# TimingSpace/MVOScaleRecovery

Hardware: AMD Instinct MI355X
Metric: frames/sec scale-recovery, KITTI-00 flow (~2k feats/frame), 1/2/4/8 GPU (higher is better)
Workload: dtype f64

## Files before the change

### mvoscalerecovery_amd/csrc/mvosr_kernels.hip

```cpp
#include <hip/hip_runtime.h>
#include <math.h>
#include <stdint.h>
#include <stdlib.h>
#include <string.h>

#include "../../include/mvosr.h"
#include "mvosr_device.hpp"
#include "mvosr_host.hpp"

namespace mvosr {

#ifdef MVOSR_STAMPS
#define MVOSR_STAMP(i) do { if (threadIdx.x == 0 && stamps) stamps[i] = __builtin_amdgcn_s_memtime(); } while (0)
#define MVOSR_STAMP_DECL unsigned long long stamps[12] = {0,0,0,0,0,0,0,0,0,0,0,0};
#define MVOSR_STAMP_ARG , unsigned long long *stamps = nullptr
#define MVOSR_STAMP_PASS , stamps
#define MVOSR_RSTAMP(i) do { if (stamps) stamps[i] = __builtin_amdgcn_s_memtime(); } while (0)
#else
#define MVOSR_RSTAMP(i) do {} while (0)
#define MVOSR_STAMP(i) do {} while (0)
#define MVOSR_STAMP_DECL
#define MVOSR_STAMP_ARG
#define MVOSR_STAMP_PASS
#endif

struct LdsPlan {
    uint32_t p, y, c, hist, red, misc, total;
// ... 22 lines not shown
    uint32_t *sel;
    int *hist;
    double *red;
    int *misc;
};
__device__ __forceinline__ Smem carve(char *base, int n, int waves) {
    const LdsPlan p = lds_plan(n, waves);
    Smem s;
    s.P = reinterpret_cast<double2 *>(base + p.p);
    s.Y = reinterpret_cast<double *>(base + p.y);
    s.c16 = reinterpret_cast<uint16_t *>(base + p.c);
    s.c32 = reinterpret_cast<uint32_t *>(base + p.c);
    s.sel = reinterpret_cast<uint32_t *>(base + p.c);
    s.hist = reinterpret_cast<int *>(base + p.hist);
    s.red = reinterpret_cast<double *>(base + p.red);
    s.misc = reinterpret_cast<int *>(base + p.misc);
    return s;
}

enum { M_WCNT = 0 , M_LIST = 16, M_MEDLO = 18, M_MEDHI = 20  };


constexpr int kTC = 2;


typedef double dvec2 __attribute__((ext_vector_type(2)));
__device__ __forceinline__ double2 stream_load2(const double2 *p) {
    const dvec2 v = __builtin_nontemporal_load(reinterpret_cast<const dvec2 *>(p));
    double2 r; r.x = v.x; r.y = v.y;
    return r;
}
__device__ __forceinline__ double stream_load(const double *p) {
    return __builtin_nontemporal_load(p);
}

template <int B>
struct TriChunk {
    TriIds q[kTC];
    template <bool STREAM = false>
    __device__ __forceinline__ void load(const int32_t *tri, int64_t begin, int count, int base, int tid) {
#pragma unroll
        for (int k = 0; k < kTC; ++k) {
            const int t = base + k * B + tid;
            if (t < count) {
                if constexpr (STREAM) {
                    const int32_t *p = tri + 3 * begin + 3 * t;
                    q[k].a = __builtin_nontemporal_load(p); q[k].b = __builtin_nontemporal_load(p + 1); q[k].c = __builtin_nontemporal_load(p + 2);
                } else {
                    q[k] = load_tri(tri + 3 * begin, t);
                }
            }
        }
    }
};

struct VoteFlags { bool f0, f1, f2; };
__device__ __forceinline__ VoteFlags vote_flags(bool pa, bool pb, bool pc, bool fixed) {
    const bool pb1 = pb & !fixed, pb2 = pb & fixed;
    VoteFlags r;
    r.f0 = pa | pb; r.f1 = pa | pb1 | pc; r.f2 = pb2 | pc;
    return r;
}
__device__ __forceinline__ int tri_rows(const int64_t *off, const int32_t *cnt, int64_t f) {
    return cnt ? cnt[f] : (int)(off[f + 1] - off[f]);
}

template <int WAVES, int SC>
__device__ __forceinline__ int phase_vote(const Smem &s, int n, const double *gx, const double *gy, const double *gz,
                                          const double *gv, const int32_t *tri1, int64_t t1_begin, int t1_count,
                                          double cp, double sp, int32_t *g_counters, int &bad,
                                          const int32_t *tri2, int64_t t2_begin, int t2_count, TriChunk<WAVES * kWave> &next,
                                          bool fixed MVOSR_STAMP_ARG) {
    constexpr int B = WAVES * kWave;
    const int tid = threadIdx.x;
    const int npad2 = (n + 1) >> 1;
    TriChunk<B> tc;
    tc.template load<true>(tri1, t1_begin, t1_count, 0, tid);
    const double2 *gy2 = reinterpret_cast<const double2 *>(gy);
    const double2 *gz2 = reinterpret_cast<const double2 *>(gz);
    const double2 *gv2 = reinterpret_cast<const double2 *>(gv);
    double2 *sY2 = reinterpret_cast<double2 *>(s.Y);
    const uint32_t ones = ((uint32_t)(kCounterBias + 1) << 16) | (uint32_t)(kCounterBias + 1);
    for (int i0 = tid; i0 < npad2; i0 += 2 * B) {
        const int i1 = i0 + B;
        const bool two = i1 < npad2;
        const double2 ya = stream_load2(gy2 + i0), za = stream_load2(gz2 + i0), va = stream_load2(gv2 + i0);
        double2 yb = ya, zb = za, vb = va;
        if (two) { yb = stream_load2(gy2 + i1); zb = stream_load2(gz2 + i1); vb = stream_load2(gv2 + i1); }
        double2 yr, p0, p1;
        yr.x = ya.x * cp - za.x * sp;  yr.y = ya.y * cp - za.y * sp;
        p0.x = va.x; p0.y = ya.x * sp + za.x * cp;
        p1.x = va.y; p1.y = ya.y * sp + za.y * cp;
        sY2[i0] = yr; s.P[2 * i0] = p0; s.P[2 * i0 + 1] = p1; s.c32[i0] = ones;
        if (two) {
            yr.x = yb.x * cp - zb.x * sp;  yr.y = yb.y * cp - zb.y * sp;
            p0.x = vb.x; p0.y = yb.x * sp + zb.x * cp;
            p1.x = vb.y; p1.y = yb.y * sp + zb.y * cp;
            sY2[i1] = yr; s.P[2 * i1] = p0; s.P[2 * i1 + 1] = p1; s.c32[i1] = ones;
        }
    }
    __syncthreads();
    MVOSR_STAMP(1);

    const int w = wave_id(), lane = lane_id();
    const int begin = w * (SC * kWave);
    double xs[SC];
#pragma unroll
    for (int k = 0; k < SC; ++k) {
        const int i = begin + k * kWave + lane;
        xs[k] = (gx && i < n) ? stream_load(gx + i) : 0.0;
    }

    TriChunk<B> tn;
    for (int base = 0; base < t1_count; base += kTC * B) {
        const bool more = base + kTC * B < t1_count;
        if (more) tn.template load<true>(tri1, t1_begin, t1_count, base + kTC * B, tid);
        double2 vp[kTC][3];
        bool vok[kTC];
#pragma unroll
        for (int k = 0; k < kTC; ++k) {
            const TriIds q = tc.q[k];
            vok[k] = base + k * B + tid < t1_count;
            if (vok[k] && ((unsigned)q.a >= (unsigned)n || (unsigned)q.b >= (unsigned)n || (unsigned)q.c >= (unsigned)n)) { bad = 1; vok[k] = false; }
            if (vok[k]) { vp[k][0] = s.P[q.a]; vp[k][1] = s.P[q.b]; vp[k][2] = s.P[q.c]; }
        }
#pragma unroll
        for (int k = 0; k < kTC; ++k) {
            if (!vok[k]) continue;
            const TriIds q = tc.q[k];
            const double2 p0 = vp[k][0], p1 = vp[k][1], p2 = vp[k][2];
            const bool pa = (p0.x - p1.x) * (p0.y - p1.y) > 0.0;
            const bool pb = (p0.x - p2.x) * (p0.y - p2.y) > 0.0;
            const bool pc = (p1.x - p2.x) * (p1.y - p2.y) > 0.0;
            const VoteFlags vf = vote_flags(pa, pb, pc, fixed);
            const bool f0 = vf.f0, f1 = vf.f1, f2 = vf.f2;
            atomicAdd(&s.c32[q.a >> 1], (f0 ? 0xFFFFFFFFu : 1u) << ((q.a & 1) * 16));
            atomicAdd(&s.c32[q.b >> 1], (f1 ? 0xFFFFFFFFu : 1u) << ((q.b & 1) * 16));
            atomicAdd(&s.c32[q.c >> 1], (f2 ? 0xFFFFFFFFu : 1u) << ((q.c & 1) * 16));
        }
        if (more) tc = tn;
    }
    if (tri2) next.load(tri2, t2_begin, t2_count, 0, tid);
    __syncthreads();
    MVOSR_STAMP(2);

    unsigned keepmask = 0u;
    double yk[SC], zk[SC];
    int cnt = 0;
#pragma unroll
    for (int k = 0; k < SC; ++k) {
        const int i = begin + k * kWave + lane;
        bool keep = false;
        yk[k] = 0.0; zk[k] = 0.0;
        if (i < n) {
            const int c = (int)s.c16[i] - kCounterBias;
            keep = c >= 0;
            if (g_counters) g_counters[i] = c;
            yk[k] = s.Y[i];
            zk[k] = s.P[i].y;
        }
        if (keep) keepmask |= 1u << k;
        cnt += __popcll(__ballot(keep));
    }
    if (lane == 0) s.misc[M_WCNT + w] = cnt;
    __syncthreads();
// ... 110 lines not shown
    for (int lo = kNpBufSize; lo < n; lo += kNpBufSize) res += np_pairwise_chunk_stream(st, min(kNpBufSize, n - lo));
    return res;
}

template <bool INLINE>
__device__ int pitch_reference_impl(double x0, double y0, double z0, double x1, double y1, double z1,
                                    double x2, double y2, double z2, double thr_deg,
                                    double &nx, double &ny, double &nz, double &pitch) {
    int r = 0;
    if (!plane_normal(x0, y0, z0, x1, y1, z1, x2, y2, z2, nx, ny, nz)) r |= 4;
    const double len2 = (nx * nx + ny * ny) + nz * nz;
    const double len = sqrt(len2);
    const double uy = ny / len;
    pitch = asin(-uy) * 180.0 / 3.141592653589793;
    if (pitch < thr_deg) r |= 1;
    if (pitch >= thr_deg) r |= 2;
    return r;
}
__device__ __attribute__((noinline)) int pitch_reference_cold(double x0, double y0, double z0, double x1, double y1, double z1,
                                                              double x2, double y2, double z2, double thr_deg) {
    double nx, ny, nz, pitch;
    return pitch_reference_impl<false>(x0, y0, z0, x1, y1, z1, x2, y2, z2, thr_deg, nx, ny, nz, pitch);
}
template <bool FULL>
__device__ __forceinline__ int pitch_reference(double x0, double y0, double z0, double x1, double y1, double z1,
                                               double x2, double y2, double z2, double thr_deg,
                                               double &nx, double &ny, double &nz, double &pitch) {
    if constexpr (FULL) return pitch_reference_impl<true>(x0, y0, z0, x1, y1, z1, x2, y2, z2, thr_deg, nx, ny, nz, pitch);
    else { nx = ny = nz = pitch = 0.0; return pitch_reference_cold(x0, y0, z0, x1, y1, z1, x2, y2, z2, thr_deg); }
}

struct SelectResult {
    double height_level;
    int n_pitch, n_tri_valid;
    int singular, bad;
    int n_steep;
    int near;
};

enum { MODE_HOT = 0, MODE_EXACT = 1, MODE_FULL = 2 };

struct PitchTest {
    double thr_deg;
    double s2_hi, s2_lo;
};

template <bool FULL>
__device__ __forceinline__ int classify_triangle(double x0, double y0, double z0, double x1, double y1, double z1,
                                                 double x2, double y2, double z2, double h, const PitchTest &pt,
                                                 double *g_normals, double *g_pitch, double *g_heights, int64_t tg) {
    bool is_flat = false, is_steep = false, is_singular = false;
    bool decided = false;
    if constexpr (!FULL) {
        const double e1x = x1 - x0, e1y = y1 - y0, e1z = z1 - z0;
        const double e2x = x2 - x0, e2y = y2 - y0, e2z = z2 - z0;
        const double cx = __builtin_fma(e1y, e2z, -(e1z * e2y));
        const double cy = __builtin_fma(e1z, e2x, -(e1x * e2z));
        const double cz = __builtin_fma(e1x, e2y, -(e1y * e2x));
        const double tx = x0 * cx, ty = y0 * cy, tz = z0 * cz;
        const double det = (tx + ty) + tz;
        const double mag = (fabs(tx) + fabs(ty)) + fabs(tz);
        const double c2 = __builtin_fma(cz, cz, __builtin_fma(cy, cy, cx * cx));
        const double q2 = cy * cy;
        const double sy = cy * det;
        const bool safe = fabs(det) > 1e-9 * mag;
        is_flat = safe & (sy > 0.0) & (q2 > pt.s2_hi * c2);
        is_steep = safe & ((sy <= 0.0) | (q2 < pt.s2_lo * c2));
        decided = is_flat | is_steep;
    }
    if (!decided) {
        double nx, ny, nz, pitch;
        const int r = pitch_reference<FULL>(x0, y0, z0, x1, y1, z1, x2, y2, z2, pt.thr_deg, nx, ny, nz, pitch);
        is_singular = r & 4;
        is_flat = r & 1;
        is_steep = r & 2;
        if constexpr (FULL) {
            if (g_normals) { double *o = g_normals + 3 * tg; o[0] = nx; o[1] = ny; o[2] = nz; }
            if (g_pitch) g_pitch[tg] = pitch;
            if (g_heights) g_heights[tg] = h;
        }
    }
    return (is_flat ? 1 : 0) | (is_steep ? 2 : 0) | (is_singular ? 4 : 0) | (decided ? 0 : 8);
}

template <bool FULL, class Fetch>
struct SteepStream {
    const int32_t *tri;
    const int32_t *order;
    int t2n;
    const PitchTest &pt;
    Fetch fetch;
    int t_next;
    unsigned long long mask;
    double h;
    __device__ __forceinline__ void refill() {
// ... 99 lines not shown
            *slot = c0 == 0 ? val[0] : *slot + val[0];
        }
        __syncthreads();
    }
    res = *slot;
    __syncthreads();
    return (0.0 + res) / (double)n_steep;
}

struct LdsFetch {
    const double2 *P; const double *Y; int n_valid;
    __device__ __forceinline__ bool operator()(const TriIds q, double &x0, double &y0, double &z0, double &x1, double &y1, double &z1,
                                               double &x2, double &y2, double &z2) const {
        if ((unsigned)q.a >= (unsigned)n_valid || (unsigned)q.b >= (unsigned)n_valid || (unsigned)q.c >= (unsigned)n_valid) return false;
        const double2 p0 = P[q.a], p1 = P[q.b], p2 = P[q.c];
        x0 = p0.x; z0 = p0.y; x1 = p1.x; z1 = p1.y; x2 = p2.x; z2 = p2.y;
        y0 = Y[q.a]; y1 = Y[q.b]; y2 = Y[q.c];
        return true;
    }
};

constexpr double kLevelGuard = 1e-12;

template <int WAVES, int MODE, int FW = 1>
__device__ __forceinline__ SelectResult phase_select(const Smem &s, int n_valid, const int32_t *tri2, int64_t t2_begin,
                                                     int t2_count, TriChunk<WAVES * kWave> &tc, PitchTest pt,
                                                     double *g_normals, double *g_pitch, double *g_heights, int bad_in,
                                                     double *scratch, int scratch_cap MVOSR_STAMP_ARG) {
    constexpr int B = WAVES * kWave;
    constexpr bool FULL = MODE == MODE_FULL;
    const int tid = threadIdx.x;
    unsigned long long flat = 0ull;
    unsigned long long flat_hi = 0ull;
    double hsum = 0.0, hcnt = 0.0, habs = 0.0;
    int npitch = 0, singular = 0, bad = 0;
    int undecided = 0;
    if (t2_count > 64 * FW * B) { bad = 1; t2_count = 0; }
    auto test_triangle = [&](int t, int kk, const TriIds q) {
    if ((unsigned)q.a >= (unsigned)n_valid || (unsigned)q.b >= (unsigned)n_valid || (unsigned)q.c >= (unsigned)n_valid) { bad = 1; return; }
    const double2 p0 = s.P[q.a], p1 = s.P[q.b], p2 = s.P[q.c];
    const double y0 = s.Y[q.a], y1 = s.Y[q.b], y2 = s.Y[q.c];
    const double x0 = p0.x, z0 = p0.y, x1 = p1.x, z1 = p1.y, x2 = p2.x, z2 = p2.y;
    const double h = MODE == MODE_HOT ? (y0 + y1) + y2 : div3((y0 + y1) + y2);
    const int r = classify_triangle<FULL>(x0, y0, z0, x1, y1, z1, x2, y2, z2, h, pt, g_normals, g_pitch, g_heights, t2_begin + t);
    const bool is_flat = r & 1, is_steep = r & 2;
    if (r & 4) singular = 1;
    if constexpr (MODE == MODE_HOT) { if (r & 8) undecided = 1; }
    if (is_steep) { hsum += h; hcnt += 1.0; if constexpr (MODE == MODE_HOT) habs += fabs(h); }
    if (is_flat) {
        if (FW == 1 || kk < 64) flat |= 1ull << (kk & 63); else flat_hi |= 1ull << (kk & 63);
        ++npitch;
    }
    };
    TriChunk<B> tn;
    for (int base = 0; base < t2_count; base += kTC * B) {
        const bool more = base + kTC * B < t2_count;
        if (more) tn.load(tri2, t2_begin, t2_count, base + kTC * B, tid);
#pragma unroll
        for (int k = 0; k < kTC; ++k) {
            const int t = base + k * B + tid;
            if (t < t2_count) test_triangle(t, base / B + k, tc.q[k]);
        }
        if (more) tc = tn;
    }
    const bool in_regs = t2_count <= kTC * B;
    if (!in_regs && t2_count > 0) tc.template load<true>(tri2, t2_begin, t2_count, 0, tid);
    if constexpr (MODE == MODE_HOT) block_sum3<WAVES>(hsum, hcnt, habs, s.red + R_SEL_H * 2 * WAVES, s.red + R_SEL_ABS * 2 * WAVES);
    else block_sum2<WAVES>(hsum, hcnt, s.red + R_SEL_H * 2 * WAVES);
    MVOSR_STAMP(4);
    SelectResult r;
    double hl = hsum / hcnt;
    const double guard = kLevelGuard * (habs / hcnt);
    if constexpr (MODE != MODE_HOT) {
        if (scratch && (int)hcnt + kNpMaxLeaves <= scratch_cap)
            hl = exact_height_level_block<WAVES, FULL>(tri2 + 3 * t2_begin, t2_count, (int)hcnt, pt, LdsFetch{s.P, s.Y, n_valid}, nullptr,
                                                       scratch, s.misc + M_WCNT, s.red + R_MISC * 2 * WAVES);
        else
            hl = exact_height_level<FULL>(tri2 + 3 * t2_begin, t2_count, (int)hcnt, pt, LdsFetch{s.P, s.Y, n_valid});
    }
    int ntv = 0, near = undecided;
    auto mark_triangle = [&](int kk, int qa, int qb, int qc) {
        const unsigned long long fw = (FW == 1 || kk < 64) ? flat : flat_hi;
        if (!((fw >> (kk & 63)) & 1ull)) return;
        const double y0 = s.Y[qa], y1 = s.Y[qb], y2 = s.Y[qc];
        const double h = MODE == MODE_HOT ? (y0 + y1) + y2 : div3((y0 + y1) + y2);
        if constexpr (MODE == MODE_HOT) { if (fabs(h - hl) <= guard) near = 1; }
        if (h > hl) {
            ++ntv;
            atomicOr(&s.sel[qa >> 5], 1u << (qa & 31));
            atomicOr(&s.sel[qb >> 5], 1u << (qb & 31));
            atomicOr(&s.sel[qc >> 5], 1u << (qc & 31));
        }
    };
    for (int base = 0; base < t2_count; base += kTC * B) {
        const bool more = base + kTC * B < t2_count;
        if (more) tn.template load<true>(tri2, t2_begin, t2_count, base + kTC * B, tid);
#pragma unroll
        for (int k = 0; k < kTC; ++k) {
            if (base + k * B + tid < t2_count) mark_triangle(base / B + k, tc.q[k].a, tc.q[k].b, tc.q[k].c);
        }
        if (more) tc = tn;
    }
    bad |= bad_in;
    int sn = singular | (near << 16);
    block_sum4i<WAVES>(npitch, ntv, sn, bad, s.red + R_SEL_CNT * 2 * WAVES);
    singular = sn & 0xFFFF;
    r.near = sn >> 16;
    MVOSR_STAMP(5);
    r.height_level = MODE == MODE_HOT ? hl / 3.0 : hl;
    r.n_steep = (int)hcnt;
    r.n_pitch = npitch; r.n_tri_valid = ntv; r.singular = singular; r.bad = bad;
    return r;
}

struct RoadResult {
    double height;
    int status;
    int n_sel, n_kept, n_modes, mode_left, mode_right;
    double mean, std, skew, median;
};

__device__ __forceinline__ bool dropped_by_single(double y, int bin, const Bits192 &single, int first_single) {
    bool d = false;
#pragma unroll
// ... 477 lines not shown
        if (a.o.stats) { double *st = a.o.stats + 4 * f; st[0] = st[1] = st[2] = st[3] = nan(""); }
    }
}

template <int MODE, bool LIST, class Body>
__device__ __forceinline__ void for_frames(const KArgs &a, Body body) {
    if constexpr (MODE == MODE_EXACT) {
        if (a.redo_pass) {
            const int count = a.redo[0];
            for (int i = blockIdx.x; i < count; i += gridDim.x) {
                body((int64_t)a.redo[1 + i]);
                __syncthreads();
            }
            return;
        }
    }
    if constexpr (LIST) {
        if ((int)blockIdx.x < *a.cls_cnt) body((int64_t)a.cls_list[blockIdx.x]);
        return;
    }
    body(a.first_frame + blockIdx.x);
}

template <int WAVES, int SC, int MODE, bool LIST = false>
__global__ __launch_bounds__(WAVES *kWave, (WAVES == 8 && MODE == MODE_HOT ? 6 : 1)) void scale_frames_kernel(const KArgs a) {
    extern __shared__ __attribute__((aligned(16))) char smem[];
    for_frames<MODE, LIST>(a, [&](const int64_t f) {
    constexpr int B = WAVES * kWave;
    MVOSR_STAMP_DECL
    MVOSR_STAMP(11);
    const int n = a.b.feat_cnt[f];
    const int64_t off = a.b.feat_off[f];
    const int64_t t1b = a.b.tri1_off[f], t2b = a.b.tri2_off[f];
    const int t1n = tri_rows(a.b.tri1_off, a.b.tri1_cnt, f), t2n = tri_rows(a.b.tri2_off, a.b.tri2_cnt, f);
    const Smem s = carve(smem, n, WAVES);
#ifdef MVOSR_STAMPS
    if (n < 0) return;
#endif
    MVOSR_STAMP(0);
#ifdef MVOSR_STAMPS
    if (threadIdx.x == 0) {
        stamps[10] = (unsigned long long)__builtin_amdgcn_s_getreg((31 << 11) | 4) | ((unsigned long long)__builtin_amdgcn_s_getreg((31 << 11) | 20) << 32);
    }
#endif

    RoadResult R;
    R.height = nan(""); R.n_sel = R.n_kept = R.n_modes = 0; R.mode_left = R.mode_right = -1;
    R.mean = R.std = R.skew = R.median = nan("");
    if (early_frame_exit(a, f, n, t2n)) return;
    int bad = 0;
    TriChunk<B> tc2;
    const int nvalid = phase_vote<WAVES, SC>(s, n, a.b.x + off, a.b.y + off, a.b.z + off, a.b.v + off, a.b.tri1, t1b, t1n,
                                             a.P.cos_pitch, a.P.sin_pitch,
                                             a.o.vote_counters ? a.o.vote_counters + off : nullptr, bad,
                                             a.b.tri2, t2b, t2n, tc2, a.P.vote_mode == MVOSR_VOTE_FIXED MVOSR_STAMP_PASS);
    const bool mask_mismatch = a.b.n2_expected && a.b.n2_expected[f] != nvalid;

    SelectResult S;
    S.height_level = nan(""); S.n_pitch = S.n_tri_valid = 0; S.singular = 0; S.bad = 1; S.n_steep = 0; S.near = 0;
    const bool too_many_rows = t1n > kMaxVoteRows;
    if (!mask_mismatch && !too_many_rows)
        S = phase_select<WAVES, MODE>(s, nvalid, a.b.tri2, t2b, t2n, tc2, a.pt, a.o.tri_normals, a.o.tri_pitch_deg,
                                      a.o.tri_heights, bad, a.ysel ? a.ysel + off : nullptr, n MVOSR_STAMP_PASS);
    frame_tail<WAVES, MODE>(a, s, f, off, nvalid, mask_mismatch || too_many_rows, S, R);
    MVOSR_STAMP(9);
#ifdef MVOSR_STAMPS
    if (threadIdx.x == 0 && a.o.hist) { unsigned long long *d = reinterpret_cast<unsigned long long *>(a.o.hist + f * 2 * kBins); for (int i = 0; i < 12; ++i) d[i] = stamps[i]; }
#endif
    });
}

struct DenseWs { double2 *P2; double *Y2; };

__host__ __device__ inline uint32_t dense_lds_bytes(int n, int waves) {
    const uint32_t npad = (uint32_t)((n + 1) & ~1);
    return align16(2u * npad + 16u) + align16(4u * ((uint32_t)(n + 31) / 32u)) + 8u * (uint32_t)(kRedSlots * 2 * waves) + 4u * 32u;
}

template <int DW, bool FUSED>
__device__ __forceinline__ int phase_vote_dense(uint32_t *c32, int *misc, int n, const double *gx, const double *gy, const double *gz,
                                                const double *gv, const int32_t *tri1, int64_t t1_begin, int t1_count,
                                                double cp, double sp, int32_t *g_counters, int &bad,
                                                double2 *P2, double *Y2, bool fixed) {
    constexpr int B = DW * kWave;
    const int tid = threadIdx.x, w = wave_id(), lane = lane_id();
// ... 83 lines not shown
    RoadResult R;
    R.height = nan(""); R.n_sel = R.n_kept = R.n_modes = 0; R.mode_left = R.mode_right = -1;
    R.mean = R.std = R.skew = R.median = nan("");
    if (early_frame_exit(a, f, n, t2n)) return;
    const uint32_t npad = (uint32_t)((n + 1) & ~1);
    Smem s;
    s.c32 = reinterpret_cast<uint32_t *>(smem);
    s.c16 = reinterpret_cast<uint16_t *>(smem);
    s.sel = reinterpret_cast<uint32_t *>(smem + align16(2u * npad + 16u));
    s.red = reinterpret_cast<double *>(smem + align16(2u * npad + 16u) + align16(4u * ((uint32_t)(n + 31) / 32u)));
    s.misc = reinterpret_cast<int *>(s.red + kRedSlots * 2 * DW);
    s.hist = nullptr;
    s.P = da.ws.P2 + off;
    s.Y = da.ws.Y2 + off;
    for (int i = tid; i < (n + 31) / 32; i += B) s.sel[i] = 0u;
    int bad = 0;
    const int nvalid = phase_vote_dense<DW, true>(s.c32, s.misc, n, a.b.x + off, a.b.y + off, a.b.z + off, a.b.v + off, a.b.tri1, t1b, t1n,
                                              a.P.cos_pitch, a.P.sin_pitch, a.o.vote_counters ? a.o.vote_counters + off : nullptr, bad,
                                              da.ws.P2 + off, da.ws.Y2 + off, a.P.vote_mode == MVOSR_VOTE_FIXED);
    const bool mask_mismatch = a.b.n2_expected && a.b.n2_expected[f] != nvalid;
    SelectResult S;
    S.height_level = nan(""); S.n_pitch = S.n_tri_valid = 0; S.singular = 0; S.bad = 1; S.n_steep = 0; S.near = 0;
    if (!mask_mismatch) {
        TriChunk<B> tc2;
        tc2.load(a.b.tri2, t2b, t2n, 0, tid);
        S = phase_select<DW, MODE, 2>(s, nvalid, a.b.tri2, t2b, t2n, tc2, a.pt, a.o.tri_normals, a.o.tri_pitch_deg,
                                      a.o.tri_heights, bad, nullptr, 0);
    }
    frame_tail<DW, MODE>(a, s, f, off, nvalid, mask_mismatch, S, R);
    });
}

template <int DW, int MODE>
__global__ __launch_bounds__(DW *kWave) void scale_frames_dense_feat_kernel(const DenseArgs da) {
    extern __shared__ __attribute__((aligned(16))) char smem[];
    const KArgs &a = da.k;
    for_frames<MODE, false>(a, [&](const int64_t f) {
    constexpr int B = DW * kWave;
    constexpr bool FULL = MODE == MODE_FULL;
    const int tid = threadIdx.x, w = wave_id(), lane = lane_id();
    const int n = a.b.feat_cnt[f];
    const int64_t off = a.b.feat_off[f];
    const int64_t t1b = a.b.tri1_off[f], t2b = a.b.tri2_off[f];
    const int t1n = tri_rows(a.b.tri1_off, a.b.tri1_cnt, f), t2n = tri_rows(a.b.tri2_off, a.b.tri2_cnt, f);
    RoadResult R;
    R.height = nan(""); R.n_sel = R.n_kept = R.n_modes = 0; R.mode_left = R.mode_right = -1;
    R.mean = R.std = R.skew = R.median = nan("");
// ... 574 lines not shown
    const int nvalid = phase_vote_dense<DW, false>(c32, misc, n, nullptr, a.b.y + off, a.b.z + off, a.b.v + off, a.b.tri1, t1b, t1n,
                                               a.P.cos_pitch, a.P.sin_pitch, a.o.vote_counters + off, bad,
                                               nullptr, nullptr, a.P.vote_mode == MVOSR_VOTE_FIXED);
    int b0 = bad, b1 = 0, b2 = 0, b3 = 0;
    block_sum4i<DW>(b0, b1, b2, b3, red + R_MISC * 2 * DW);
    if (threadIdx.x == 0) {
        if (a.o.counts) a.o.counts[f * MVOSR_N_COUNTS + MVOSR_CNT_VALID] = nvalid;
        if (a.o.status) a.o.status[f] = b0 ? MVOSR_ST_ERR_MASK : MVOSR_ST_MODE;
    }
}

template <int WAVES, int SC>
__global__ __launch_bounds__(WAVES *kWave) void outlier_vote_kernel(const KArgs a) {
    extern __shared__ __attribute__((aligned(16))) char smem[];
    const int64_t f = a.first_frame + blockIdx.x;
    const int n = a.b.feat_cnt[f];
    if (n <= 0) { if (threadIdx.x == 0 && a.o.counts) a.o.counts[f * MVOSR_N_COUNTS + MVOSR_CNT_VALID] = 0; return; }
    const int64_t off = a.b.feat_off[f];
    const int64_t t1b = a.b.tri1_off[f];
    const int t1n = tri_rows(a.b.tri1_off, a.b.tri1_cnt, f);
    const Smem s = carve(smem, n, WAVES);
    int bad = 0;
    MVOSR_STAMP_DECL
    TriChunk<WAVES * kWave> unused;
    const int nvalid = phase_vote<WAVES, SC>(s, n, nullptr, a.b.y + off, a.b.z + off, a.b.v + off, a.b.tri1, t1b, t1n,
                                             a.P.cos_pitch, a.P.sin_pitch, a.o.vote_counters + off, bad, nullptr, 0, 0, unused,
                                             a.P.vote_mode == MVOSR_VOTE_FIXED MVOSR_STAMP_PASS);
    int b0 = bad | (t1n > kMaxVoteRows ? 1 : 0), b1 = 0, b2 = 0, b3 = 0;
    block_sum4i<WAVES>(b0, b1, b2, b3, s.red + R_MISC * 2 * WAVES);
    if (threadIdx.x == 0) {
        if (a.o.counts) a.o.counts[f * MVOSR_N_COUNTS + MVOSR_CNT_VALID] = nvalid;
        if (a.o.status) a.o.status[f] = b0 ? MVOSR_ST_ERR_MASK : MVOSR_ST_MODE;
    }
}

constexpr int kMaxWindow = 64;
struct MedianArgs {
    const double *raw; double *out; int64_t n; int window; int n_queue;
    int n_blocks; int64_t base_len, extra, stride;
    double queue[kMaxWindow];
};
__device__ __forceinline__ double median_seq_at(const MedianArgs &a, int64_t i) {
    if (a.n_blocks <= 1) return a.raw[i];
    const int64_t head = a.extra * (a.base_len + 1);
    int64_t r, j;
    if (i < head) { r = i / (a.base_len + 1); j = i - r * (a.base_len + 1); }
    else { const int64_t k = i - head; r = a.extra + k / a.base_len; j = k - (r - a.extra) * a.base_len; }
// ... 28 lines not shown
template <typename K>
static int prepare_kernel(K kernel, size_t lds) {
    hipError_t e = hipFuncSetAttribute(reinterpret_cast<const void *>(kernel), hipFuncAttributeMaxDynamicSharedMemorySize, (int)lds);
    if (e != hipSuccess) return set_hip_error("hipFuncSetAttribute(MaxDynamicSharedMemorySize)", e);
    return MVOSR_OK;
}

static PitchTest make_pitch_test(double thr_deg) {
    PitchTest pt;
    pt.thr_deg = thr_deg;
    if (thr_deg < -1.0 && thr_deg > -89.9) {
        const double sn = sin(-thr_deg * 3.141592653589793 / 180.0);
        pt.s2_hi = sn * sn * (1.0 + 1e-9);
        pt.s2_lo = sn * sn * (1.0 - 1e-9);
    } else {
        pt.s2_hi = INFINITY;
        pt.s2_lo = -INFINITY;
    }
    return pt;
}

constexpr int kClassHeader = 4;
constexpr int kWaves1Max = 320, kWaves4Max = 1152;
constexpr int kClassThr0 = kWaves1Max, kClassThr1 = 1024;
constexpr int64_t kClassMinFrames = 2048;
constexpr int32_t kClassHintMagic = 0x4d56;
constexpr int kClassifyWaves = 16;
struct ClassArgs {
    const int32_t *feat_cnt;
    int64_t first_frame, n_frames;
    int32_t *hdr;
    int32_t *lists;
    int64_t stride;
    int32_t *redo;
    int grid[3];
};

__host__ __device__ inline int size_class_of(int n) { return n <= kClassThr0 ? 0 : (n <= kClassThr1 ? 1 : 2); }

__global__ __launch_bounds__(kClassifyWaves *kWave) void classify_frames_kernel(const ClassArgs c) {
    __shared__ int wcnt[kClassifyWaves][3];
    __shared__ int bbase[3];
    const int64_t i = blockIdx.x * (int64_t)blockDim.x + threadIdx.x;
    const int lane = threadIdx.x & (kWave - 1), w = threadIdx.x / kWave;
    int cls = -1;
    int32_t f = 0;
    if (i < c.n_frames) {
        f = (int32_t)(c.first_frame + i);
        cls = size_class_of(c.feat_cnt[f]);
    }
    const uint64_t m0 = __ballot(cls == 0), m1 = __ballot(cls == 1), m2 = __ballot(cls == 2);
    if (lane == 0) { wcnt[w][0] = __popcll(m0); wcnt[w][1] = __popcll(m1); wcnt[w][2] = __popcll(m2); }
    __syncthreads();
    if (threadIdx.x < 3) {
        int tot = 0;
        for (int ww = 0; ww < kClassifyWaves; ++ww) tot += wcnt[ww][threadIdx.x];
        bbase[threadIdx.x] = tot ? atomicAdd(c.hdr + threadIdx.x, tot) : 0;
    }
    __syncthreads();
    if (cls < 0) return;
    const uint64_t m = cls == 0 ? m0 : (cls == 1 ? m1 : m2);
    int pos = bbase[cls] + __popcll(m & ((1ull << lane) - 1ull));
    for (int ww = 0; ww < w; ++ww) pos += wcnt[ww][cls];
    if (pos < c.grid[cls]) c.lists[cls * c.stride + pos] = f;
    else c.redo[1 + atomicAdd(c.redo, 1)] = f;
}

static int pick_waves(int requested, int max_feat) {
    if (requested == 1 || requested == 4 || requested == 8 || requested == 16) return requested;
    if (max_feat <= kWaves1Max) return 1;
    if (max_feat <= kWaves4Max) return 4;
    if (max_feat <= 2048 || 2 * (int64_t)lds_plan(max_feat, 8).total <= (int64_t)g_max_dyn_lds) return 8;
    return 16;
}
static int variant_capacity(int waves, int sc) { return waves * sc * kWave; }
static int lds_capacity_features() {
    int lo = 1, hi = variant_capacity(16, 8);
    while (lo < hi) {
        const int mid = (lo + hi + 1) / 2;
        if ((int64_t)lds_plan(mid, 16).total <= (int64_t)g_max_dyn_lds) lo = mid; else hi = mid - 1;
    }
    return lo;
}

static int check_common(mvosr_ctx *ctx, const mvosr_params *p, const mvosr_batch *b, const mvosr_outputs *o) {
    if (!ctx || !p || !b || !o) return set_error(MVOSR_ERR_ARG, "null argument");
    if (b->n_frames < 0 || !b->feat_off || !b->feat_cnt) return set_error(MVOSR_ERR_ARG, "batch without frames/offsets");
    if (b->max_feat < 0) return set_error(MVOSR_ERR_ARG, "max_feat < 0");
    return MVOSR_OK;
}

static int check_fit(const mvosr_batch *b, int waves, int sc, size_t lds) {
    if ((int64_t)lds > (int64_t)g_max_dyn_lds)
        return set_error(MVOSR_ERR_TOO_LARGE, "frame of %d features needs %zu B of LDS (> %d)", b->max_feat, lds, g_max_dyn_lds);
    if (b->max_feat > variant_capacity(waves, sc))
        return set_error(MVOSR_ERR_TOO_LARGE, "%d features exceed what %d wavefronts per frame handle (%d)", b->max_feat, waves,
                         variant_capacity(waves, sc));
    if ((int64_t)2 * b->max_feat > (int64_t)64 * kWave * waves)
// ... 39 lines not shown
        kargs_of(args).redo_pass = 1;
        const unsigned grid = (unsigned)(nl < (int64_t)kRedoGrid ? nl : (int64_t)kRedoGrid);
        hipLaunchKernelGGL(k_exact, dim3(grid), dim3(threads), lds, ctx_stream(ctx), args);
        return check_launch(name);
    }
    if (mode == MODE_EXACT) {
        hipLaunchKernelGGL(k_exact, dim3((unsigned)nl), dim3(threads), lds, ctx_stream(ctx), args);
        return check_launch(name);
    }
    if ((rc = prepare_kernel(k_hot, lds_hot))) return rc;
    const hipError_t e = hipMemsetAsync(kargs_of(args).redo, 0, sizeof(int32_t), ctx_stream(ctx));
    if (e != hipSuccess) return set_hip_error("hipMemsetAsync(redo list)", e);
    hipLaunchKernelGGL(k_hot, dim3((unsigned)nl), dim3(threads_hot), lds_hot, ctx_stream(ctx), args);
    if ((rc = check_launch(name))) return rc;
    if (!g_hot_only && (rc = launch_append_mask(ctx, kargs_of(args), nl, true))) return rc;
    return MVOSR_OK;
}

template <int WAVES, int SC>
static int launch_scale(mvosr_ctx *ctx, const KArgs &ka, int64_t nl, int mode) {
    const size_t lds = lds_plan(ka.b.max_feat, WAVES).total;
    int rc = check_fit(&ka.b, WAVES, SC, lds);
    if (rc) return rc;
    return launch_modes<KArgs>(ctx, scale_frames_kernel<WAVES, SC, MODE_HOT>, scale_frames_kernel<WAVES, SC, MODE_EXACT>,
                               scale_frames_kernel<WAVES, SC, MODE_FULL>, ka, nl, WAVES * kWave, lds, mode, "scale_frames_kernel");
}

template <int WAVES, int SC>
static int launch_vote(mvosr_ctx *ctx, const KArgs &ka, int64_t nl) {
    const size_t lds = lds_plan(ka.b.max_feat, WAVES).total;
    int rc = check_fit(&ka.b, WAVES, SC, lds);
    if (rc) return rc;
    if ((rc = prepare_kernel(outlier_vote_kernel<WAVES, SC>, lds))) return rc;
    hipLaunchKernelGGL((outlier_vote_kernel<WAVES, SC>), dim3((unsigned)nl), dim3(WAVES * kWave), lds, ctx_stream(ctx), ka);
    return check_launch("outlier_vote_kernel");
}

constexpr int kDenseWaves = 16;

template <int DW>
static int launch_scale_dense_w(mvosr_ctx *ctx, const KArgs &ka, int64_t nl, int mode, bool vote_only) {
    if ((int64_t)2 * ka.b.max_feat > (int64_t)128 * kWave * DW)
        return set_error(MVOSR_ERR_TOO_LARGE, "%d features give more triangles than %d wavefronts sweep", ka.b.max_feat, DW);
    const size_t lds = dense_lds_bytes(ka.b.max_feat, DW);
    if ((int64_t)lds > (int64_t)g_max_dyn_lds)
        return set_error(MVOSR_ERR_TOO_LARGE, "frame of %d features needs %zu B of LDS (> %d)", ka.b.max_feat, lds, g_max_dyn_lds);
    DenseArgs da;
// ... 40 lines not shown
    if (ra.list) hipLaunchKernelGGL(road_model_kernel<true>, dim3(blocks), dim3(kRoadWaves * kWave), 0, stream, ra);
    else hipLaunchKernelGGL(road_model_kernel<false>, dim3(blocks), dim3(kRoadWaves * kWave), 0, stream, ra);
    return check_launch("road_model_kernel");
}

#define MVOSR_DISPATCH(FN, ...)                                                             \
    do {                                                                                    \
        const int n_ = ka.b.max_feat;                                                       \
        switch (waves) {                                                                    \
            case 1: return FN<1, 8>(__VA_ARGS__);                                           \
            case 4: return (n_ <= variant_capacity(4, 4)) ? FN<4, 4>(__VA_ARGS__) : FN<4, 8>(__VA_ARGS__);     \
            case 16: return (n_ <= variant_capacity(16, 4)) ? FN<16, 4>(__VA_ARGS__) : FN<16, 8>(__VA_ARGS__); \
            default: return (n_ <= variant_capacity(8, 4)) ? FN<8, 4>(__VA_ARGS__) : FN<8, 8>(__VA_ARGS__);    \
        }                                                                                   \
    } while (0)

static int dispatch_scale(mvosr_ctx *ctx, const KArgs &ka, int waves, int64_t nl, int mode) { MVOSR_DISPATCH(launch_scale, ctx, ka, nl, mode); }
static int dispatch_vote(mvosr_ctx *ctx, const KArgs &ka, int waves, int64_t nl) { MVOSR_DISPATCH(launch_vote, ctx, ka, nl); }

typedef void (*scale_kernel_fn)(const KArgs);
static scale_kernel_fn hot_list_kernel(int waves, int n) {
    switch (waves) {
        case 1: return scale_frames_kernel<1, 8, MODE_HOT, true>;
        case 4: return (n <= variant_capacity(4, 4)) ? scale_frames_kernel<4, 4, MODE_HOT, true> : scale_frames_kernel<4, 8, MODE_HOT, true>;
        case 16: return (n <= variant_capacity(16, 4)) ? scale_frames_kernel<16, 4, MODE_HOT, true> : scale_frames_kernel<16, 8, MODE_HOT, true>;
        default: return (n <= variant_capacity(8, 4)) ? scale_frames_kernel<8, 4, MODE_HOT, true> : scale_frames_kernel<8, 8, MODE_HOT, true>;
    }
}

static int launch_scale_classes(mvosr_ctx *ctx, const KArgs &ka, int64_t nl) {
    int rc;
    hipError_t e;
    int32_t *hdr = ka.nsel + 3 * ka.b.n_frames + 4;
    ClassArgs ca;
    ca.feat_cnt = ka.b.feat_cnt; ca.first_frame = ka.first_frame; ca.n_frames = nl;
    ca.hdr = hdr; ca.lists = hdr + kClassHeader; ca.stride = ka.b.n_frames; ca.redo = ka.redo;
    const bool hinted = ka.b.size_hint[3] == kClassHintMagic;
    const int thr[3] = {kClassThr0, kClassThr1, ka.b.max_feat};
    scale_kernel_fn fn[3];
    int waves[3];
    size_t lds[3];
    KArgs kc[3];
    for (int c = 0; c < 3; ++c) {
        kc[c] = ka;
        kc[c].b.max_feat = thr[c] < ka.b.max_feat ? thr[c] : ka.b.max_feat;
        const int n = kc[c].b.max_feat;
        waves[c] = pick_waves(0, n);
// ... 262 lines not shown
```

Before: 27.09 million.

## Add register-resident packed triangle rows variant for large-frame HOT kernel

```diff
diff --git a/mvoscalerecovery_amd/csrc/mvosr_kernels.hip b/mvoscalerecovery_amd/csrc/mvosr_kernels.hip
--- a/mvoscalerecovery_amd/csrc/mvosr_kernels.hip
+++ b/mvoscalerecovery_amd/csrc/mvosr_kernels.hip
@@ -3,6 +3,8 @@
 #include <stdint.h>
 #include <stdlib.h>
 #include <string.h>
+
+#include <type_traits>
 
 #include "../../include/mvosr.h"
 #include "mvosr_device.hpp"
@@ -71,6 +73,7 @@
 
 
 constexpr int kTC = 2;
+constexpr int kTCFat = 4;
 
 
 typedef double dvec2 __attribute__((ext_vector_type(2)));
@@ -83,13 +86,13 @@
     return __builtin_nontemporal_load(p);
 }
 
-template <int B>
+template <int B, int TC>
 struct TriChunk {
-    TriIds q[kTC];
+    TriIds q[TC];
     template <bool STREAM = false>
     __device__ __forceinline__ void load(const int32_t *tri, int64_t begin, int count, int base, int tid) {
 #pragma unroll
-        for (int k = 0; k < kTC; ++k) {
+        for (int k = 0; k < TC; ++k) {
             const int t = base + k * B + tid;
             if (t < count) {
                 if constexpr (STREAM) {
@@ -101,6 +104,57 @@
             }
         }
     }
+    __device__ __forceinline__ void first(const int32_t *tri, int64_t begin, int count, int tid) { load(tri, begin, count, 0, tid); }
+};
+
+constexpr int kResRows = 16;
+template <int B>
+struct ResidentRows {
+    TriIds raw[kResRows];
+    __device__ __forceinline__ void first(const int32_t *tri, int64_t begin, int count, int tid) {
+        const int32_t *rows = tri + 3 * begin;
+#pragma unroll
+        for (int k = 0; k < kResRows; ++k) {
+            const int t = k * B + tid;
+            if (t < count) raw[k] = load_tri(rows, t);
+        }
+    }
+};
+struct PackedRows {
+    uint32_t w[3 * kResRows / 2];
+    uint32_t live;
+    template <int B>
+    __device__ __forceinline__ void pack(const ResidentRows<B> &r, int count, int n_valid, int tid, int &bad) {
+        uint32_t there = 0u;
+        live = 0u;
+#pragma unroll
+        for (int j = 0; j < kResRows / 2; ++j) {
+            uint32_t id[6];
+#pragma unroll
+            for (int h = 0; h < 2; ++h) {
+                const int k = 2 * j + h;
+                const TriIds q = r.raw[k];
+                const bool present = k * B + tid < count;
+                const bool legal = present && (unsigned)q.a < (unsigned)n_valid && (unsigned)q.b < (unsigned)n_valid && (unsigned)q.c < (unsigned)n_valid;
+                if (present) there |= 1u << k;
+                if (legal) live |= 1u << k;
+                id[3 * h] = legal ? (uint32_t)q.a : 0u;
+                id[3 * h + 1] = legal ? (uint32_t)q.b : 0u;
+                id[3 * h + 2] = legal ? (uint32_t)q.c : 0u;
+            }
+            w[3 * j] = id[0] | (id[1] << 16); w[3 * j + 1] = id[2] | (id[3] << 16); w[3 * j + 2] = id[4] | (id[5] << 16);
+        }
+        if (there != live) bad = 1;
+    }
+    __device__ __forceinline__ void pin(int k) {
+        const int j = 3 * (k / 2) + (k % 2);
+        asm volatile("" : "+v"(w[j]), "+v"(w[j + 1]));
+    }
+    __device__ __forceinline__ void ids(int k, int &a, int &b, int &c) const {
+        const int j = 3 * (k / 2);
+        if (k % 2 == 0) { a = (int)(w[j] & 0xFFFFu); b = (int)(w[j] >> 16); c = (int)(w[j + 1] & 0xFFFFu); }
+        else { a = (int)(w[j + 1] >> 16); b = (int)(w[j + 2] & 0xFFFFu); c = (int)(w[j + 2] >> 16); }
+    }
 };
 
 struct VoteFlags { bool f0, f1, f2; };
@@ -114,22 +168,43 @@
     return cnt ? cnt[f] : (int)(off[f + 1] - off[f]);
 }
 
-template <int WAVES, int SC>
+template <int WAVES, int SC, int TC = kTC, int FU = 2, class Next = TriChunk<WAVES * kWave, kTC>>
 __device__ __forceinline__ int phase_vote(const Smem &s, int n, const double *gx, const double *gy, const double *gz,
                                           const double *gv, const int32_t *tri1, int64_t t1_begin, int t1_count,
                                           double cp, double sp, int32_t *g_counters, int &bad,
-                                          const int32_t *tri2, int64_t t2_begin, int t2_count, TriChunk<WAVES * kWave> &next,
+                                          const int32_t *tri2, int64_t t2_begin, int t2_count, Next &next,
                                           bool fixed MVOSR_STAMP_ARG) {
     constexpr int B = WAVES * kWave;
     const int tid = threadIdx.x;
     const int npad2 = (n + 1) >> 1;
-    TriChunk<B> tc;
+    TriChunk<B, TC> tc;
     tc.template load<true>(tri1, t1_begin, t1_count, 0, tid);
     const double2 *gy2 = reinterpret_cast<const double2 *>(gy);
     const double2 *gz2 = reinterpret_cast<const double2 *>(gz);
     const double2 *gv2 = reinterpret_cast<const double2 *>(gv);
     double2 *sY2 = reinterpret_cast<double2 *>(s.Y);
     const uint32_t ones = ((uint32_t)(kCounterBias + 1) << 16) | (uint32_t)(kCounterBias + 1);
+    if constexpr (FU != 2) {
+        for (int i0 = tid; i0 < npad2; i0 += FU * B) {
+            double2 yv[FU], zv[FU], vv[FU];
+#pragma unroll
+            for (int u = 0; u < FU; ++u) {
+                const int i = i0 + u * B;
+                if (i < npad2) { yv[u] = stream_load2(gy2 + i); zv[u] = stream_load2(gz2 + i); vv[u] = stream_load2(gv2 + i); }
+            }
+#pragma unroll
+            for (int u = 0; u < FU; ++u) {
+                const int i = i0 + u * B;
+                if (i < npad2) {
+                    double2 yr, p0, p1;
+                    yr.x = yv[u].x * cp - zv[u].x * sp;  yr.y = yv[u].y * cp - zv[u].y * sp;
+                    p0.x = vv[u].x; p0.y = yv[u].x * sp + zv[u].x * cp;
+                    p1.x = vv[u].y; p1.y = yv[u].y * sp + zv[u].y * cp;
+                    sY2[i] = yr; s.P[2 * i] = p0; s.P[2 * i + 1] = p1; s.c32[i] = ones;
+                }
+            }
+        }
+    } else
     for (int i0 = tid; i0 < npad2; i0 += 2 * B) {
         const int i1 = i0 + B;
         const bool two = i1 < npad2;
@@ -160,21 +235,25 @@
         xs[k] = (gx && i < n) ? stream_load(gx + i) : 0.0;
     }
 
-    TriChunk<B> tn;
-    for (int base = 0; base < t1_count; base += kTC * B) {
-        const bool more = base + kTC * B < t1_count;
-        if (more) tn.template load<true>(tri1, t1_begin, t1_count, base + kTC * B, tid);
-        double2 vp[kTC][3];
-        bool vok[kTC];
-#pragma unroll
-        for (int k = 0; k < kTC; ++k) {
+    TriChunk<B, TC> tn;
+    for (int base = 0; base < t1_count; base += TC * B) {
+        const bool more = base + TC * B < t1_count;
+        if (more) tn.template load<true>(tri1, t1_begin, t1_count, base + TC * B, tid);
+        double2 vp[TC][3];
+        bool vok[TC];
+#pragma unroll
+        for (int k = 0; k < TC; ++k) {
             const TriIds q = tc.q[k];
             vok[k] = base + k * B + tid < t1_count;
             if (vok[k] && ((unsigned)q.a >= (unsigned)n || (unsigned)q.b >= (unsigned)n || (unsigned)q.c >= (unsigned)n)) { bad = 1; vok[k] = false; }
-            if (vok[k]) { vp[k][0] = s.P[q.a]; vp[k][1] = s.P[q.b]; vp[k][2] = s.P[q.c]; }
-        }
-#pragma unroll
-        for (int k = 0; k < kTC; ++k) {
+            if constexpr (TC == kTC) {
+                if (vok[k]) { vp[k][0] = s.P[q.a]; vp[k][1] = s.P[q.b]; vp[k][2] = s.P[q.c]; }
+            } else {
+                vp[k][0] = s.P[vok[k] ? q.a : 0]; vp[k][1] = s.P[vok[k] ? q.b : 0]; vp[k][2] = s.P[vok[k] ? q.c : 0];
+            }
+        }
+#pragma unroll
+        for (int k = 0; k < TC; ++k) {
             if (!vok[k]) continue;
             const TriIds q = tc.q[k];
             const double2 p0 = vp[k][0], p1 = vp[k][1], p2 = vp[k][2];
@@ -189,7 +268,7 @@
         }
         if (more) tc = tn;
     }
-    if (tri2) next.load(tri2, t2_begin, t2_count, 0, tid);
+    if (tri2) next.first(tri2, t2_begin, t2_count, tid);
     __syncthreads();
     MVOSR_STAMP(2);
 
@@ -346,11 +425,12 @@
     double nx, ny, nz, pitch;
     return pitch_reference_impl<false>(x0, y0, z0, x1, y1, z1, x2, y2, z2, thr_deg, nx, ny, nz, pitch);
 }
-template <bool FULL>
+template <bool FULL, bool COLD_INLINE = false>
 __device__ __forceinline__ int pitch_reference(double x0, double y0, double z0, double x1, double y1, double z1,
                                                double x2, double y2, double z2, double thr_deg,
                                                double &nx, double &ny, double &nz, double &pitch) {
-    if constexpr (FULL) return pitch_reference_impl<true>(x0, y0, z0, x1, y1, z1, x2, y2, z2, thr_deg, nx, ny, nz, pitch);
+    if constexpr (COLD_INLINE) return pitch_reference_impl<false>(x0, y0, z0, x1, y1, z1, x2, y2, z2, thr_deg, nx, ny, nz, pitch);
+    else if constexpr (FULL) return pitch_reference_impl<true>(x0, y0, z0, x1, y1, z1, x2, y2, z2, thr_deg, nx, ny, nz, pitch);
     else { nx = ny = nz = pitch = 0.0; return pitch_reference_cold(x0, y0, z0, x1, y1, z1, x2, y2, z2, thr_deg); }
 }
 
@@ -369,10 +449,10 @@
     double s2_hi, s2_lo;
 };
 
-template <bool FULL>
+template <bool FULL, bool COLD_INLINE = false>
 __device__ __forceinline__ int classify_triangle(double x0, double y0, double z0, double x1, double y1, double z1,
                                                  double x2, double y2, double z2, double h, const PitchTest &pt,
-                                                 double *g_normals, double *g_pitch, double *g_heights, int64_t tg) {
+                                                 double *g_normals, double *g_pitch, double *g_heights, int64_t tg, bool cold = true) {
     bool is_flat = false, is_steep = false, is_singular = false;
     bool decided = false;
     if constexpr (!FULL) {
@@ -392,9 +472,9 @@
         is_steep = safe & ((sy <= 0.0) | (q2 < pt.s2_lo * c2));
         decided = is_flat | is_steep;
     }
-    if (!decided) {
+    if (!decided && cold) {
         double nx, ny, nz, pitch;
-        const int r = pitch_reference<FULL>(x0, y0, z0, x1, y1, z1, x2, y2, z2, pt.thr_deg, nx, ny, nz, pitch);
+        const int r = pitch_reference<FULL, COLD_INLINE>(x0, y0, z0, x1, y1, z1, x2, y2, z2, pt.thr_deg, nx, ny, nz, pitch);
         is_singular = r & 4;
         is_flat = r & 1;
         is_steep = r & 2;
@@ -540,9 +620,64 @@
 
 constexpr double kLevelGuard = 1e-12;
 
-template <int WAVES, int MODE, int FW = 1>
+struct RowVerts { double2 p0, p1, p2; double y0, y1, y2; };
+__device__ __forceinline__ void resident_gather(const Smem &s, PackedRows &rows, int k, RowVerts &v) {
+    int a, b, c;
+    rows.pin(k);
+    rows.ids(k, a, b, c);
+    v.p0 = s.P[a]; v.p1 = s.P[b]; v.p2 = s.P[c];
+    v.y0 = s.Y[a]; v.y1 = s.Y[b]; v.y2 = s.Y[c];
+}
+constexpr int kResAhead = 1;
+__device__ __forceinline__ bool resident_first_sweep(const Smem &s, PackedRows &rows, const PitchTest &pt, double *h3,
+                                                     unsigned long long &flat, int &npitch, double &hsum, double &hcnt, double &habs) {
+    uint32_t flat_bits = 0u;
+    int undecided = 0;
+    RowVerts ring[kResAhead + 1];
+#pragma unroll
+    for (int k = 0; k < kResAhead; ++k) resident_gather(s, rows, k, ring[k]);
+#pragma unroll
+    for (int k = 0; k < kResRows; ++k) {
+        if (k + kResAhead < kResRows) resident_gather(s, rows, k + kResAhead, ring[(k + kResAhead) % (kResAhead + 1)]);
+        RowVerts &cur = ring[k % (kResAhead + 1)];
+        asm volatile("" : "+v"(cur.p0.x), "+v"(cur.p0.y), "+v"(cur.p1.x), "+v"(cur.p1.y), "+v"(cur.p2.x), "+v"(cur.p2.y),
+                          "+v"(cur.y0), "+v"(cur.y1), "+v"(cur.y2) : : "memory");
+        const bool live = (rows.live >> k) & 1u;
+        double h = (cur.y0 + cur.y1) + cur.y2;
+        int r = classify_triangle<false>(cur.p0.x, cur.y0, cur.p0.y, cur.p1.x, cur.y1, cur.p1.y, cur.p2.x, cur.y2, cur.p2.y, h, pt,
+                                         nullptr, nullptr, nullptr, 0, false);
+        r = live ? r : 0;
+        if (r & 8) undecided = 1;
+        if (r & 2) { hsum += h; hcnt += 1.0; habs += fabs(h); }
+        if (r & 1) { flat_bits |= 1u << k; ++npitch; }
+        asm volatile("" : "+v"(h), "+v"(hsum), "+v"(hcnt), "+v"(habs), "+v"(flat_bits), "+v"(npitch), "+v"(undecided));
+        h3[k] = h;
+        __builtin_amdgcn_sched_barrier(0);
+    }
+    flat = flat_bits;
+    return undecided != 0;
+}
+__device__ __forceinline__ void resident_second_sweep(const Smem &s, const PackedRows &rows, const double *h3, unsigned long long flat,
+                                                      double hl, double guard, int &near, int &ntv) {
+#pragma unroll
+    for (int k = 0; k < kResRows; ++k) {
+        if (!((flat >> k) & 1ull)) continue;
+        const double h = h3[k];
+        if (fabs(h - hl) <= guard) near = 1;
+        if (h > hl) {
+            int a, b, c;
+            rows.ids(k, a, b, c);
+            ++ntv;
+            atomicOr(&s.sel[a >> 5], 1u << (a & 31));
+            atomicOr(&s.sel[b >> 5], 1u << (b & 31));
+            atomicOr(&s.sel[c >> 5], 1u << (c & 31));
+        }
+    }
+}
+
+template <int WAVES, int MODE, int FW = 1, int TC = kTC, bool RES = false, class First = TriChunk<WAVES * kWave, TC>>
 __device__ __forceinline__ SelectResult phase_select(const Smem &s, int n_valid, const int32_t *tri2, int64_t t2_begin,
-                                                     int t2_count, TriChunk<WAVES * kWave> &tc, PitchTest pt,
+                                                     int t2_count, First &first, PitchTest pt,
                                                      double *g_normals, double *g_pitch, double *g_heights, int bad_in,
                                                      double *scratch, int scratch_cap MVOSR_STAMP_ARG) {
     constexpr int B = WAVES * kWave;
@@ -554,13 +689,13 @@
     int npitch = 0, singular = 0, bad = 0;
     int undecided = 0;
     if (t2_count > 64 * FW * B) { bad = 1; t2_count = 0; }
-    auto test_triangle = [&](int t, int kk, const TriIds q) {
+    auto test_triangle = [&](int t, int kk, const TriIds q, auto cold_inline) {
     if ((unsigned)q.a >= (unsigned)n_valid || (unsigned)q.b >= (unsigned)n_valid || (unsigned)q.c >= (unsigned)n_valid) { bad = 1; return; }
     const double2 p0 = s.P[q.a], p1 = s.P[q.b], p2 = s.P[q.c];
     const double y0 = s.Y[q.a], y1 = s.Y[q.b], y2 = s.Y[q.c];
     const double x0 = p0.x, z0 = p0.y, x1 = p1.x, z1 = p1.y, x2 = p2.x, z2 = p2.y;
     const double h = MODE == MODE_HOT ? (y0 + y1) + y2 : div3((y0 + y1) + y2);
-    const int r = classify_triangle<FULL>(x0, y0, z0, x1, y1, z1, x2, y2, z2, h, pt, g_normals, g_pitch, g_heights, t2_begin + t);
+    const int r = classify_triangle<FULL, decltype(cold_inline)::value>(x0, y0, z0, x1, y1, z1, x2, y2, z2, h, pt, g_normals, g_pitch, g_heights, t2_begin + t);
     const bool is_flat = r & 1, is_steep = r & 2;
     if (r & 4) singular = 1;
     if constexpr (MODE == MODE_HOT) { if (r & 8) undecided = 1; }
@@ -570,19 +705,35 @@
         ++npitch;
     }
     };
-    TriChunk<B> tn;
-    for (int base = 0; base < t2_count; base += kTC * B) {
-        const bool more = base + kTC * B < t2_count;
-        if (more) tn.load(tri2, t2_begin, t2_count, base + kTC * B, tid);
-#pragma unroll
-        for (int k = 0; k < kTC; ++k) {
+    static_assert(!RES || (MODE == MODE_HOT && FW == 1 && kResRows % 2 == 0 && kResRows < 64), "the resident form is a HOT variant");
+    TriChunk<B, TC> tn;
+    PackedRows rows;
+    double h3[RES ? kResRows : 1];
+    int k_streamed = kResRows;
+    if constexpr (RES) {
+        rows.pack(first, t2_count, n_valid, tid, bad);
+        if (resident_first_sweep(s, rows, pt, h3, flat, npitch, hsum, hcnt, habs)) {
+            k_streamed = 0;
+            flat = 0ull; npitch = 0; hsum = hcnt = habs = 0.0;
+        }
+#pragma unroll 1
+        for (int k = k_streamed; k * B + tid < t2_count; ++k)
+            test_triangle(k * B + tid, k, load_tri(tri2 + 3 * t2_begin, k * B + tid), std::true_type{});
+    } else {
+    TriChunk<B, TC> &tc = first;
+    for (int base = 0; base < t2_count; base += TC * B) {
+        const bool more = base + TC * B < t2_count;
+        if (more) tn.load(tri2, t2_begin, t2_count, base + TC * B, tid);
+#pragma unroll
+        for (int k = 0; k < TC; ++k) {
             const int t = base + k * B + tid;
-            if (t < t2_count) test_triangle(t, base / B + k, tc.q[k]);
+            if (t < t2_count) test_triangle(t, base / B + k, tc.q[k], std::false_type{});
         }
         if (more) tc = tn;
     }
-    const bool in_regs = t2_count <= kTC * B;
+    const bool in_regs = t2_count <= TC * B;
     if (!in_regs && t2_count > 0) tc.template load<true>(tri2, t2_begin, t2_count, 0, tid);
+    }
     if constexpr (MODE == MODE_HOT) block_sum3<WAVES>(hsum, hcnt, habs, s.red + R_SEL_H * 2 * WAVES, s.red + R_SEL_ABS * 2 * WAVES);
     else block_sum2<WAVES>(hsum, hcnt, s.red + R_SEL_H * 2 * WAVES);
     MVOSR_STAMP(4);
@@ -610,14 +761,24 @@
             atomicOr(&s.sel[qc >> 5], 1u << (qc & 31));
         }
     };
-    for (int base = 0; base < t2_count; base += kTC * B) {
-        const bool more = base + kTC * B < t2_count;
-        if (more) tn.template load<true>(tri2, t2_begin, t2_count, base + kTC * B, tid);
-#pragma unroll
-        for (int k = 0; k < kTC; ++k) {
+    if constexpr (RES) {
+        if (k_streamed != 0) resident_second_sweep(s, rows, h3, flat, hl, guard, near, ntv);
+#pragma unroll 1
+        for (int k = k_streamed; k * B + tid < t2_count; ++k) {
+            const TriIds q = load_tri(tri2 + 3 * t2_begin, k * B + tid);
+            mark_triangle(k, q.a, q.b, q.c);
+        }
+    } else {
+    TriChunk<B, TC> &tc = first;
+    for (int base = 0; base < t2_count; base += TC * B) {
+        const bool more = base + TC * B < t2_count;
+        if (more) tn.template load<true>(tri2, t2_begin, t2_count, base + TC * B, tid);
+#pragma unroll
+        for (int k = 0; k < TC; ++k) {
             if (base + k * B + tid < t2_count) mark_triangle(base / B + k, tc.q[k].a, tc.q[k].b, tc.q[k].c);
         }
         if (more) tc = tn;
+    }
     }
     bad |= bad_in;
     int sn = singular | (near << 16);
@@ -1141,11 +1302,14 @@
     body(a.first_frame + blockIdx.x);
 }
 
-template <int WAVES, int SC, int MODE, bool LIST = false>
-__global__ __launch_bounds__(WAVES *kWave, (WAVES == 8 && MODE == MODE_HOT ? 6 : 1)) void scale_frames_kernel(const KArgs a) {
+template <int WAVES, int SC, int MODE, bool LIST = false, bool RES = false>
+__global__ __launch_bounds__(WAVES *kWave, (RES ? 3 : WAVES == 8 && MODE == MODE_HOT ? 6 : 1)) void scale_frames_kernel(const KArgs a) {
+    static_assert(!RES || (WAVES == 4 && SC == 8 && MODE == MODE_HOT), "the resident form is <4, 8, HOT>");
     extern __shared__ __attribute__((aligned(16))) char smem[];
     for_frames<MODE, LIST>(a, [&](const int64_t f) {
     constexpr int B = WAVES * kWave;
+    constexpr int TC = RES ? kTCFat : kTC, FU = RES ? 4 : 2;
+    using Rows2 = typename std::conditional<RES, ResidentRows<B>, TriChunk<B, TC>>::type;
     MVOSR_STAMP_DECL
     MVOSR_STAMP(11);
     const int n = a.b.feat_cnt[f];
@@ -1168,8 +1332,8 @@
     R.mean = R.std = R.skew = R.median = nan("");
     if (early_frame_exit(a, f, n, t2n)) return;
     int bad = 0;
-    TriChunk<B> tc2;
-    const int nvalid = phase_vote<WAVES, SC>(s, n, a.b.x + off, a.b.y + off, a.b.z + off, a.b.v + off, a.b.tri1, t1b, t1n,
+    Rows2 tc2;
+    const int nvalid = phase_vote<WAVES, SC, TC, FU>(s, n, a.b.x + off, a.b.y + off, a.b.z + off, a.b.v + off, a.b.tri1, t1b, t1n,
                                              a.P.cos_pitch, a.P.sin_pitch,
                                              a.o.vote_counters ? a.o.vote_counters + off : nullptr, bad,
                                              a.b.tri2, t2b, t2n, tc2, a.P.vote_mode == MVOSR_VOTE_FIXED MVOSR_STAMP_PASS);
@@ -1179,7 +1343,7 @@
     S.height_level = nan(""); S.n_pitch = S.n_tri_valid = 0; S.singular = 0; S.bad = 1; S.n_steep = 0; S.near = 0;
     const bool too_many_rows = t1n > kMaxVoteRows;
     if (!mask_mismatch && !too_many_rows)
-        S = phase_select<WAVES, MODE>(s, nvalid, a.b.tri2, t2b, t2n, tc2, a.pt, a.o.tri_normals, a.o.tri_pitch_deg,
+        S = phase_select<WAVES, MODE, 1, TC, RES>(s, nvalid, a.b.tri2, t2b, t2n, tc2, a.pt, a.o.tri_normals, a.o.tri_pitch_deg,
                                       a.o.tri_heights, bad, a.ysel ? a.ysel + off : nullptr, n MVOSR_STAMP_PASS);
     frame_tail<WAVES, MODE>(a, s, f, off, nvalid, mask_mismatch || too_many_rows, S, R);
     MVOSR_STAMP(9);
@@ -1309,7 +1473,7 @@
     SelectResult S;
     S.height_level = nan(""); S.n_pitch = S.n_tri_valid = 0; S.singular = 0; S.bad = 1; S.n_steep = 0; S.near = 0;
     if (!mask_mismatch) {
-        TriChunk<B> tc2;
+        TriChunk<B, kTC> tc2;
         tc2.load(a.b.tri2, t2b, t2n, 0, tid);
         S = phase_select<DW, MODE, 2>(s, nvalid, a.b.tri2, t2b, t2n, tc2, a.pt, a.o.tri_normals, a.o.tri_pitch_deg,
                                       a.o.tri_heights, bad, nullptr, 0);
@@ -1930,7 +2094,7 @@
     const Smem s = carve(smem, n, WAVES);
     int bad = 0;
     MVOSR_STAMP_DECL
-    TriChunk<WAVES * kWave> unused;
+    TriChunk<WAVES * kWave, kTC> unused;
     const int nvalid = phase_vote<WAVES, SC>(s, n, nullptr, a.b.y + off, a.b.z + off, a.b.v + off, a.b.tri1, t1b, t1n,
                                              a.P.cos_pitch, a.P.sin_pitch, a.o.vote_counters + off, bad, nullptr, 0, 0, unused,
                                              a.P.vote_mode == MVOSR_VOTE_FIXED MVOSR_STAMP_PASS);
@@ -2005,6 +2169,7 @@
 
 constexpr int kClassHeader = 4;
 constexpr int kWaves1Max = 320, kWaves4Max = 1152;
+constexpr int kResidentMin = 1728;
 constexpr int kClassThr0 = kWaves1Max, kClassThr1 = 1024;
 constexpr int64_t kClassMinFrames = 2048;
 constexpr int32_t kClassHintMagic = 0x4d56;
@@ -2049,14 +2214,15 @@
     else c.redo[1 + atomicAdd(c.redo, 1)] = f;
 }
 
+static int variant_capacity(int waves, int sc) { return waves * sc * kWave; }
 static int pick_waves(int requested, int max_feat) {
     if (requested == 1 || requested == 4 || requested == 8 || requested == 16) return requested;
     if (max_feat <= kWaves1Max) return 1;
     if (max_feat <= kWaves4Max) return 4;
+    if (max_feat >= kResidentMin && max_feat <= variant_capacity(4, 8)) return 4;
     if (max_feat <= 2048 || 2 * (int64_t)lds_plan(max_feat, 8).total <= (int64_t)g_max_dyn_lds) return 8;
     return 16;
 }
-static int variant_capacity(int waves, int sc) { return waves * sc * kWave; }
 static int lds_capacity_features() {
     int lo = 1, hi = variant_capacity(16, 8);
     while (lo < hi) {
@@ -2142,7 +2308,9 @@
     const size_t lds = lds_plan(ka.b.max_feat, WAVES).total;
     int rc = check_fit(&ka.b, WAVES, SC, lds);
     if (rc) return rc;
-    return launch_modes<KArgs>(ctx, scale_frames_kernel<WAVES, SC, MODE_HOT>, scale_frames_kernel<WAVES, SC, MODE_EXACT>,
+    void (*k_hot)(const KArgs) = scale_frames_kernel<WAVES, SC, MODE_HOT>;
+    if constexpr (WAVES == 4 && SC == 8) { if (ka.b.max_feat >= kResidentMin) k_hot = scale_frames_kernel<4, 8, MODE_HOT, false, true>; }
+    return launch_modes<KArgs>(ctx, k_hot, scale_frames_kernel<WAVES, SC, MODE_EXACT>,
                                scale_frames_kernel<WAVES, SC, MODE_FULL>, ka, nl, WAVES * kWave, lds, mode, "scale_frames_kernel");
 }
 
@@ -2229,7 +2397,8 @@
 static scale_kernel_fn hot_list_kernel(int waves, int n) {
     switch (waves) {
         case 1: return scale_frames_kernel<1, 8, MODE_HOT, true>;
-        case 4: return (n <= variant_capacity(4, 4)) ? scale_frames_kernel<4, 4, MODE_HOT, true> : scale_frames_kernel<4, 8, MODE_HOT, true>;
+        case 4: return (n <= variant_capacity(4, 4)) ? scale_frames_kernel<4, 4, MODE_HOT, true>
+                       : (n >= kResidentMin ? scale_frames_kernel<4, 8, MODE_HOT, true, true> : scale_frames_kernel<4, 8, MODE_HOT, true>);
         case 16: return (n <= variant_capacity(16, 4)) ? scale_frames_kernel<16, 4, MODE_HOT, true> : scale_frames_kernel<16, 8, MODE_HOT, true>;
         default: return (n <= variant_capacity(8, 4)) ? scale_frames_kernel<8, 4, MODE_HOT, true> : scale_frames_kernel<8, 8, MODE_HOT, true>;
     }
```

After: 27.23 million, median of 2. No clear change (+0.5%).
